# bjzhb666/GS-LoRA

Measured on AMD Instinct MI355X. Metric: forgetting-step images/sec, ViT-P8S8 d6 112px r=8, higher is better.
Workload: dtype fp16

## Files before the change

### gs-lora_amd/csrc/gemm.hip

```cpp
#include <stdlib.h>

#include "gsl_common.h"
#include <type_traits>

using namespace gsl;
#include "gsl_h16.h"
GSL_OPNS_BEGIN

typedef op16x8_t bf16x8_t;
typedef __attribute__((ext_vector_type(4))) float f32x4_t;

struct EpiArgs {
  float alpha;
  const float* bias;
  const void* res;
  const void* aux;
  void* out;
  void* out2;
  int ldo;
  const float* pos;
  const float* cls;
  int T;
  DropCfg drop;
  int M, N;
// ... 2173 lines not shown
      return launch_gemm<GSL_EPI_MUL>(dtype, A1, lda1, W1, ldw1, K1, A2, lda2, W2, ldw2, K2, e, st);
    case GSL_EPI_BIAS_GELU_G8:
      GSL_CHECK_ARG(bias && dtype == GSL_OP16 && (N % 64) == 0, "bias required, bf16 only, N % 64 == 0 (slab-major code tensor)");
      return launch_gemm<GSL_EPI_BIAS_GELU_G8>(dtype, A1, lda1, W1, ldw1, K1, A2, lda2, W2, ldw2, K2, e, st);
    case GSL_EPI_MUL_G8:
      GSL_CHECK_ARG(aux && dtype == GSL_OP16 && (N % 64) == 0, "aux required, bf16 only, N % 64 == 0 (slab-major code tensor)");
      return launch_gemm<GSL_EPI_MUL_G8>(dtype, A1, lda1, W1, ldw1, K1, A2, lda2, W2, ldw2, K2, e, st);
    case GSL_EPI_PATCH:
      GSL_CHECK_ARG(bias && pos && cls && T > 0, "bias/pos/cls/T required");
      return launch_gemm<GSL_EPI_PATCH>(dtype, A1, lda1, W1, ldw1, K1, A2, lda2, W2, ldw2, K2, e, st);
    default: return fail(GSL_ERR_ARG, "gsl_gemm_nt: unknown epilogue%s %ld", "", epilogue);
  }
}

static int gemm_nt_lora_rows(const void* A, int lda, const void* W, int ldw, int K, const void* P, int ldp, const void* Q,
                             int ldq, float lora_scale, void* tout, int ldt, int M, int N, int dtype, int epilogue,
                             const float* bias, const void* res, const void* aux, void* out, void* out2, int ldo,
                             float p_drop, uint64_t seed, uint32_t site, gsl_stream_t s, int mbase);

extern "C" int GSL_ENTRY(gsl_gemm_nt_lora)(const void* A, int lda, const void* W, int ldw, int K, const void* P, int ldp, const void* Q,
                                int ldq, float lora_scale, void* tout, int ldt, int M, int N, int dtype, int epilogue,
                                const float* bias, const void* res, const void* aux, void* out, void* out2, int ldo,
                                float p_drop, uint64_t seed, uint32_t site, gsl_stream_t s) {
  GSL_FORWARD_H16(dtype, h16_gsl_gemm_nt_lora(A, lda, W, ldw, K, P, ldp, Q, ldq, lora_scale, tout, ldt, M, N, dtype, epilogue, bias, res, aux, out,
                                              out2, ldo, p_drop, seed, site, s));
  const bool splittable = (epilogue == GSL_EPI_STORE && !out2) || epilogue == GSL_EPI_BIAS_RES_BF16 || epilogue == GSL_EPI_BIAS_RES_F16;
  const int tail = (splittable && A && W && out && M >= 1024) ? tail_split_rows(M, N, dtype) : 0;
  if (tail > 0) {
    const int head = M - tail;
    const int rc = gemm_nt_lora_rows(A, lda, W, ldw, K, P, ldp, Q, ldq, lora_scale, tout, ldt, head, N, dtype, epilogue, bias, res, aux, out, out2, ldo,
                                     p_drop, seed, site, s, 0);
    if (rc) return rc;
    return gemm_nt_lora_rows(rows_after(A, head, lda, 2), lda, W, ldw, K, P, ldp, Q, ldq, lora_scale, rows_after(tout, head, ldt, 2), ldt, tail, N, dtype,
                             epilogue, bias, rows_after(res, head, ldo, 2), aux, rows_after(out, head, ldo, 2), out2, ldo, p_drop, seed, site, s, head);
  }
  return gemm_nt_lora_rows(A, lda, W, ldw, K, P, ldp, Q, ldq, lora_scale, tout, ldt, M, N, dtype, epilogue, bias, res, aux, out, out2, ldo, p_drop, seed,
                           site, s, 0);
}

static int gemm_nt_lora_rows(const void* A, int lda, const void* W, int ldw, int K, const void* P, int ldp, const void* Q,
                             int ldq, float lora_scale, void* tout, int ldt, int M, int N, int dtype, int epilogue,
                             const float* bias, const void* res, const void* aux, void* out, void* out2, int ldo,
                             float p_drop, uint64_t seed, uint32_t site, gsl_stream_t s, int mbase) {
  if (dtype != GSL_OP16) return fail(GSL_ERR_UNSUPPORTED, "gsl_gemm_nt_lora: bf16 / fp16 operands only (f32 parity mode uses gsl_gemm_nt with a K segment)%s %ld", "", dtype);
  GSL_CHECK_ARG(M > 0 && N > 0 && (N % 4) == 0 && K > 0 && (K % 64) == 0, "M,N>0, N%4==0, K%64==0");
  GSL_CHECK_ARG(A && W && P && Q && out, "null operand");
// ... 152 lines not shown
```

### gs-lora_amd/csrc/gsl_common.h

```cpp
#pragma once
#include <hip/hip_runtime.h>
#include <stdint.h>
#include <stdio.h>
#include <string.h>

#include "../../include/gslora_hip.h"

namespace gsl {

extern thread_local char g_err[512];
inline int fail(int code, const char* fmt, const char* a = "", long b = 0, long c = 0) {
  snprintf(g_err, sizeof(g_err), fmt, a, b, c);
  return code;
}
#define GSL_CHECK_ARG(cond, msg)                                                        \
  do {                                                                                  \
    if (!(cond)) return gsl::fail(GSL_ERR_ARG, "%s: argument check failed: " msg " (%ld,%ld)", __func__, 0, 0); \
  } while (0)
inline int check_launch(const char* what) {
  hipError_t e = hipGetLastError();
  if (e != hipSuccess) {
    snprintf(g_err, sizeof(g_err), "%s: %s", what, hipGetErrorString(e));
    return GSL_ERR_LAUNCH;
  }
// ... 195 lines not shown
__device__ __forceinline__ void drop_mul4(const DropCfg& d, uint64_t idx, float m[4]) {
  drop_mul4_w(d, d.thr ? drop_w0(d.key, idx >> 1) : 0u, m);
}

__device__ __forceinline__ float gelu_f(float x) { return 0.5f * x * (1.0f + erff(x * 0.70710678118654752f)); }
__device__ __forceinline__ float gelu_grad_f(float x) {
  const float cdf = 0.5f * (1.0f + erff(x * 0.70710678118654752f));
  const float pdf = 0.39894228040143268f * expf(-0.5f * x * x);
  return cdf + x * pdf;
}

__device__ __forceinline__ void gelu_pair_fast(float a, float& g, float& gp) {
  const float t = __builtin_amdgcn_rcpf(fmaf(fabsf(a), 0.3275911f * 0.70710678118654752f, 1.0f));
  const float e = __builtin_amdgcn_exp2f((a * a) * -0.72134752044448170f);
  const float ph = t * fmaf(t, fmaf(t, fmaf(t, fmaf(t, 0.5f * 1.061405429f, 0.5f * -1.453152027f), 0.5f * 1.421413741f), 0.5f * -0.284496736f),
                            0.5f * 0.254829592f);
  const float cdf = 0.5f + copysignf(fmaf(-ph, e, 0.5f), a);
  g = a * cdf;
  gp = fmaf(a * 0.39894228040143268f, e, cdf);
}

inline hipStream_t as_stream(gsl_stream_t s) { return reinterpret_cast<hipStream_t>(s); }

}
```

### gs-lora_amd/csrc/lora.hip

```cpp
#include "gsl_common.h"

using namespace gsl;

constexpr int LG_ROWS = 64;
constexpr int LG_FAN = 32;

template <typename T> struct LgVec;
template <> struct LgVec<bf16_t> {
  static constexpr int V = 8;
  static __device__ __forceinline__ void ld(const bf16_t* p, float v[8]) {
    const uint4 t = *reinterpret_cast<const uint4*>(p);
    v[0] = __uint_as_float(t.x << 16); v[1] = __uint_as_float(t.x & 0xffff0000u);
    v[2] = __uint_as_float(t.y << 16); v[3] = __uint_as_float(t.y & 0xffff0000u);
    v[4] = __uint_as_float(t.z << 16); v[5] = __uint_as_float(t.z & 0xffff0000u);
    v[6] = __uint_as_float(t.w << 16); v[7] = __uint_as_float(t.w & 0xffff0000u);
  }
};
template <> struct LgVec<f16_t> {
  static constexpr int V = 8;
  static __device__ __forceinline__ void ld(const f16_t* p, float v[8]) {
    const uint4 t = *reinterpret_cast<const uint4*>(p);
    unpack2h(t.x, v[0], v[1]); unpack2h(t.y, v[2], v[3]); unpack2h(t.z, v[4], v[5]); unpack2h(t.w, v[6], v[7]);
  }
};
// ... 366 lines not shown
  }
  lg_plan(M, N, V, R, CG, bx, nsplit, rps);
  const int RP = 256 / CG;
  const size_t red_bytes = (size_t)(RP - 1) * CG * V * R * sizeof(float);
  float* part2 = ws + (size_t)nsplit * N * R;
#define LAUNCH(TT, RR)                                                                                                   \
  hipLaunchKernelGGL((lora_grad_partial_kernel<TT, RR>), dim3(bx, nsplit), dim3(256), red_bytes, st, (const TT*)Y, ldy, (const TT*)U, \
                     ldu, ws, M, N, rps, CG)
  if (dtype == GSL_BF16) { if (R == 8) LAUNCH(bf16_t, 8); else LAUNCH(bf16_t, 16); }
  else if (dtype == GSL_F16) { if (R == 8) LAUNCH(f16_t, 8); else LAUNCH(f16_t, 16); }
  else { if (R == 8) LAUNCH(float, 8); else LAUNCH(float, 16); }
#undef LAUNCH
  int rc = check_launch("gsl_lora_grad(partial)");
  if (rc) return rc;
  const int tot = N * R;
  int nslab = (nsplit + LG_FAN - 1) / LG_FAN;
  if (nslab == 1) { part2 = ws; nslab = nsplit; }
  else hipLaunchKernelGGL(lora_grad_reduce1_kernel, dim3((tot + 255) / 256, nslab), dim3(256), 0, st, ws, part2, tot, nsplit);
  if (R == 8) hipLaunchKernelGGL(lora_grad_reduce2_kernel<8>, dim3((tot + 255) / 256), dim3(256), 0, st, part2, G, gsn, gsj, N, r, nslab, accumulate, gscale);
  else hipLaunchKernelGGL(lora_grad_reduce2_kernel<16>, dim3((tot + 255) / 256), dim3(256), 0, st, part2, G, gsn, gsj, N, r, nslab, accumulate, gscale);
  return check_launch("gsl_lora_grad(reduce)");
}

__global__ __launch_bounds__(256) void gnorm_partial_kernel(const float* __restrict__ flat, const int64_t* __restrict__ toff,
                                                            const int64_t* __restrict__ tnumel, float* __restrict__ partial) {
  fp16_sat_on();
  __shared__ float sm[16];
  const int t = blockIdx.x, sp = blockIdx.y;
  const int64_t n = tnumel[t];
  const float* p = flat + toff[t];
  const int64_t chunk = ((n + GSL_NORM_SPLIT - 1) / GSL_NORM_SPLIT + 3) & ~(int64_t)3;
  const int64_t b = sp * chunk, e = min(n, b + chunk);
  float acc = 0.f;
  const bool al = ((reinterpret_cast<uintptr_t>(p + b) & 15) == 0);
  if (al) {
    const int64_t n4 = (e > b) ? (e - b) / 4 : 0;
    const float4* p4 = reinterpret_cast<const float4*>(p + b);
    for (int64_t i = threadIdx.x; i < n4; i += blockDim.x) {
      const float4 v = p4[i];
      acc += v.x * v.x + v.y * v.y + v.z * v.z + v.w * v.w;
    }
    for (int64_t i = b + n4 * 4 + threadIdx.x; i < e; i += blockDim.x) acc += p[i] * p[i];
  } else {
    for (int64_t i = b + threadIdx.x; i < e; i += blockDim.x) acc += p[i] * p[i];
  }
  const float tot = block_sum(acc, sm);
// ... 285 lines not shown
```

### gs-lora_amd/csrc/norm.hip

```cpp
#include "gsl_common.h"

using namespace gsl;

template <int NPL>
struct RowIO {
  static constexpr int VEC = (NPL % 4 == 0) ? 4 : 1;
  static constexpr int NV = NPL / VEC;
  static __device__ __forceinline__ int idx(int lane, int c, int i) { return (c * 64 + lane) * VEC + i; }
  template <typename T>
  static __device__ __forceinline__ void load(const T* row, int lane, float v[NPL]) {
#pragma unroll
    for (int c = 0; c < NV; ++c) {
      if constexpr (VEC == 4) Elem<T>::ld4(row + (c * 64 + lane) * 4, &v[c * 4]);
      else v[c] = Elem<T>::ld(row + c * 64 + lane);
    }
  }
  template <typename T>
  static __device__ __forceinline__ void store(T* row, int lane, const float v[NPL]) {
#pragma unroll
    for (int c = 0; c < NV; ++c) {
      if constexpr (VEC == 4) Elem<T>::st4(row + (c * 64 + lane) * 4, &v[c * 4]);
      else Elem<T>::st(row + c * 64 + lane, v[c]);
    }
  }
// ... 54 lines not shown
#pragma unroll
      for (int i = 0; i < NPL; ++i) am = fmaxf(am, fabsf(gy[i]));
    }
#pragma unroll
    for (int i = 0; i < NPL; ++i) {
      xv[i] = (xv[i] - mu) * rs;
      gy[i] *= g[i];
      s1 += gy[i];
      s2 += gy[i] * xv[i];
    }
    const float c1 = wave_sum(s1) * (1.0f / D), c2 = wave_sum(s2) * (1.0f / D);
#pragma unroll
    for (int i = 0; i < NPL; ++i) gy[i] = rs * (gy[i] - c1 - xv[i] * c2);
    if (dres && (cls_T == 0 || (row % cls_T) == 0)) {
      float r[NPL];
      IO::load(dres + (size_t)(cls_T ? row / cls_T : row) * ios, lane, r);
#pragma unroll
      for (int i = 0; i < NPL; ++i) gy[i] += r[i];
    }
    if (gmax) {
#pragma unroll
      for (int i = 0; i < NPL; ++i) am = fmaxf(am, fabsf(gy[i]));
    }
    IO::store(dx + (size_t)row * (cls_T ? (long)D : ios), lane, gy);
    if (dxb) {
      if (drop.thr) {
#pragma unroll
        for (int c = 0; c < IO::NV; ++c) {
          if constexpr (IO::VEC == 4) {
            float dm[4];
            drop_mul4(drop, (uint64_t)row * drop_row_stride + IO::idx(lane, c, 0), dm);
#pragma unroll
            for (int i = 0; i < 4; ++i) gy[c * 4 + i] *= dm[i];
          } else {
            gy[c] *= drop_mul(drop, (uint64_t)row * drop_row_stride + IO::idx(lane, c, 0));
          }
        }
      }
      IO::store(dxb + (size_t)row * D, lane, gy);
    }
  }
  if (gmax) {
    am = wave_max(am);
    if (lane == 0 && !(am <= *gmax)) atomicMax(reinterpret_cast<unsigned int*>(gmax), __float_as_uint(am));
  }
}

// ... 132 lines not shown
    case 256: return CALL(4);                                                               \
    case 512: return CALL(8);                                                               \
    case 768: return CALL(12);                                                              \
    case 1024: return CALL(16);                                                             \
    default: return fail(GSL_ERR_UNSUPPORTED, "%s: unsupported LayerNorm width %ld", __func__, (long)(D)); \
  }

extern "C" int gsl_layernorm_fwd(const void* x, long x_row_stride, const float* gamma, const float* beta, float eps,
                                 void* y, float* mean, float* rstd, int M, int D, int dtype, int x_dtype, gsl_stream_t s) {
  GSL_CHECK_ARG(x && gamma && beta && mean && rstd && M > 0, "null/size");
  GSL_CHECK_ARG(dtype == GSL_F32 || dtype == GSL_BF16 || dtype == GSL_F16, "dtype");
  GSL_CHECK_ARG(x_dtype == GSL_F32 || ((x_dtype == GSL_BF16 || x_dtype == GSL_F16) && dtype == GSL_BF16) || (x_dtype == GSL_F16 && dtype == GSL_F16),
                "x dtype (a 16-bit stream only in a 16-bit mode; bf16 stream only with bf16 operands)");
  GSL_CHECK_ARG((x_row_stride % 4) == 0, "row stride alignment");
#define CALL(N) ln_fwd_launch<N>(x, x_row_stride, gamma, beta, eps, y, mean, rstd, M, dtype, x_dtype, as_stream(s))
  GSL_DISPATCH_D(D, CALL)
#undef CALL
}

extern "C" int gsl_layernorm_bwd(const void* dy, const void* x, long x_row_stride, const float* gamma, const float* mean,
                                 const float* rstd, const void* dres, void* dx, long io_row_stride, void* dxb, int M, int D,
                                 int dtype, int stream_dtype, int x_dtype, float p_drop, uint64_t seed, uint32_t site,
                                 long drop_row_stride, int dres_cls_T, float* gmax, gsl_stream_t s) {
  GSL_CHECK_ARG(dy && x && gamma && mean && rstd && dx && M > 0, "null/size");
  GSL_CHECK_ARG(dtype == GSL_F32 || dtype == GSL_BF16 || dtype == GSL_F16, "dtype");
  GSL_CHECK_ARG(stream_dtype == GSL_F32 || (stream_dtype == dtype && dtype != GSL_F32), "stream dtype (f32, or the operand format of a 16-bit mode)");
  GSL_CHECK_ARG(x_dtype == GSL_F32 || ((x_dtype == GSL_BF16 || x_dtype == GSL_F16) && dtype == GSL_BF16) || (x_dtype == GSL_F16 && dtype == GSL_F16),
                "x dtype (a 16-bit stream only in a 16-bit mode; bf16 stream only with bf16 operands)");
  GSL_CHECK_ARG((x_row_stride % 4) == 0, "row stride alignment");
  GSL_CHECK_ARG(dres_cls_T >= 0 && (dres_cls_T == 0 || (dres && dres != dx)), "dres_cls_T: compact dres, out of place");
  const DropCfg drop = make_drop(p_drop, seed, site);
  const long ios = io_row_stride > 0 ? io_row_stride : D, drs = drop_row_stride > 0 ? drop_row_stride : D;
  GSL_CHECK_ARG((ios % 4) == 0, "io row stride alignment");
#define CALL(N) ln_bwd_launch<N>(dy, x, x_row_stride, gamma, mean, rstd, dres, dx, ios, dxb, M, dtype, stream_dtype, x_dtype, drop, drs, dres_cls_T, gmax, as_stream(s))
  GSL_DISPATCH_D(D, CALL)
#undef CALL
}

extern "C" int gsl_layernorm_fwd_lora(const void* x, long x_row_stride, const float* gamma, const float* beta, float eps, void* y,
                                      float* mean, float* rstd, int M, int D, const void* P, int ldp, float alpha, void* u,
                                      gsl_stream_t s) {
  GSL_CHECK_ARG(x && gamma && beta && y && mean && rstd && P && u && M > 0, "null/size");
  GSL_CHECK_ARG(D == 512 || D == 768, "width (512 or 768)");
  GSL_CHECK_ARG((x_row_stride % 8) == 0 && (ldp % 8) == 0 && ldp >= D, "row stride alignment");
  const int grid = min((M + 63) / 64, 256 * 4);
  if (D == 512)
    hipLaunchKernelGGL((ln_fwd_lora_kernel<16>), dim3(grid), dim3(256), 0, as_stream(s), (const bf16_t*)x, x_row_stride, gamma, beta, eps,
// ... 7 lines not shown
```

### gs-lora_amd/gslora_hip/ops.py

```python
import ctypes

import torch

from . import _lib as L

ATTN_MAX_T = 1025


def check_num_tokens(model, T):
    if T > ATTN_MAX_T:
        raise NotImplementedError(f"{model}: this geometry gives {T} tokens per image; the gs-lora_amd attention kernels take at most "
                                  f"{ATTN_MAX_T} (GSL_ATTN_MAX_T: a 32 x 32 patch grid plus the cls token)")


DT = {torch.float32: L.F32, torch.bfloat16: L.BF16, torch.float16: L.F16}


def _p(t):
    return None if t is None else t.data_ptr()


def _stream():
    return torch.cuda.current_stream().cuda_stream

# ... 269 lines not shown
    _need(x, gamma, beta)
    mean = torch.empty(M, device=x.device, dtype=torch.float32)
    rstd = torch.empty(M, device=x.device, dtype=torch.float32)
    L.check(L.load().gsl_layernorm_fwd(_p(x), row_stride, _p(gamma), _p(beta), float(eps), None, _p(mean), _p(rstd), M, D,
                                       code(dtype), code(x.dtype), _stream()), "gsl_layernorm_fwd(stats)")
    return mean, rstd


def layernorm_fwd_lora(x, row_stride, M, D, gamma, beta, eps, P, alpha, pad=64):
    _need(x, gamma, beta, P)
    if x.dtype != torch.bfloat16 or P.dtype != torch.bfloat16 or P.shape[0] < 16 or P.shape[1] != D or pad != 64:
        raise ValueError("layernorm_fwd_lora: bf16 x, P [>= 16, D] bf16, 64-column u")
    y = torch.empty(M, D, device=x.device, dtype=torch.bfloat16)
    u = torch.empty(M, pad, device=x.device, dtype=torch.bfloat16)
    mean = torch.empty(M, device=x.device, dtype=torch.float32)
    rstd = torch.empty(M, device=x.device, dtype=torch.float32)
    L.check(L.load().gsl_layernorm_fwd_lora(_p(x), row_stride, _p(gamma), _p(beta), float(eps), _p(y), _p(mean), _p(rstd), M, D,
                                            _p(P), P.stride(0), float(alpha), _p(u), _stream()), "gsl_layernorm_fwd_lora")
    return y, mean, rstd, u


@_profiled("ln_bwd", lambda dy, *a, **k: (dy.shape[0], dy.shape[1], 0, 0))
def layernorm_bwd(dy, x, row_stride, gamma, mean, rstd, dres, want_copy=True, p_drop=0.0, seed=0, site=0, dx=None,
                  io_row_stride=0, drop_row_stride=0, dres_cls_T=0, gmax=None):
    _need(dy, x, gamma, mean, rstd)
    M, D = dy.shape
    sdt = dx.dtype if dx is not None else (dres.dtype if dres is not None else torch.float32)
    own_dx = dx is None
    if dx is None:
        _need(dres)
        dx = torch.empty(M, D, device=dy.device, dtype=sdt)
    elif dres is not None and dres.dtype != dx.dtype:
        raise RuntimeError("layernorm_bwd: dres and dx must share one dtype")
    alias = bool(want_copy) and float(p_drop) == 0.0 and sdt == dy.dtype and own_dx and not io_row_stride
    dxb = torch.empty(M, D, device=dy.device, dtype=dy.dtype) if (want_copy and not alias) else None
    L.check(L.load().gsl_layernorm_bwd(_p(dy), _p(x), row_stride, _p(gamma), _p(mean), _p(rstd), _p(dres), _p(dx),
                                       int(io_row_stride), _p(dxb), M, D, code(dy.dtype), code(sdt), code(x.dtype), float(p_drop),
                                       int(seed), int(site), int(drop_row_stride), int(dres_cls_T), _p(gmax), _stream()), "gsl_layernorm_bwd")
    return dx, (dx if alias else dxb)


@_profiled("attn_fwd", lambda qkv, B, T, H, *a, **k: (B * T, H * 64, T, H))
def attention_fwd(qkv, B, T, H, scale, layout=0):
    _need(qkv)
    o = torch.empty(B * T, H * 64, device=qkv.device, dtype=qkv.dtype)
    lse = torch.empty(B, H, T, device=qkv.device, dtype=torch.float32)
    L.check(L.load().gsl_attention_fwd(_p(qkv), _p(o), _p(lse), B, T, H, float(scale), code(qkv.dtype), int(layout), _stream()),
            "gsl_attention_fwd")
    return o, lse


@_profiled("attn_bwd", lambda qkv, o, d_o, lse, B, T, H, *a, **k: (B * T, H * 64, T, H))
def attention_bwd(qkv, o, d_o, lse, B, T, H, scale, layout=0):
    _need(qkv, o, d_o, lse)
    dqkv = torch.empty_like(qkv)
    delta = torch.empty(B, H, T, device=qkv.device, dtype=torch.float32)
    L.check(L.load().gsl_attention_bwd(_p(qkv), _p(o), _p(d_o), _p(lse), _p(dqkv), _p(delta), B, T, H, float(scale),
                                       code(qkv.dtype), int(layout), _stream()), "gsl_attention_bwd")
    return dqkv


def attention_fwd_cls(qkv, B, T, H, scale, layout=0, q_cls=None):
# ... 7 lines not shown

def attention_bwd_cls(qkv, o, d_o_cls, lse, B, T, H, scale, layout=0, q_cls=None):
    _need(qkv, o, d_o_cls, lse, q_cls)
    nw = 2 if layout == 2 else 3
    dqkv = torch.empty(B * T, nw * H * 64, device=qkv.device, dtype=qkv.dtype)
    dq = torch.empty(B, H * 64, device=qkv.device, dtype=qkv.dtype) if layout == 2 else None
    compact = o.shape[0] == B and lse.dim() == 2
    L.check(L.load().gsl_attention_bwd_cls(_p(qkv), _p(q_cls), _p(o), _p(d_o_cls), _p(lse), _p(dqkv), _p(dq), B, T, H, float(scale),
                                           code(qkv.dtype), int(layout), 1 if compact else 0, _stream()), "gsl_attention_bwd_cls")
    return (dqkv, dq) if layout == 2 else dqkv




def lora_grad(Y, U, G, gsn, gsj, r, accumulate=True, gscale=None):
    if not (Y.is_cuda and U.is_cuda and Y.stride(1) == 1 and U.stride(1) == 1):
        raise RuntimeError("lora_grad: operands must be CUDA tensors with unit column stride")
    M, N = Y.shape
    lib = L.load()
    need = lib.gsl_lora_grad_ws_elems(M, N, r)
    ws = _workspace((Y.device.index,), need, Y.device, floor=1 << 22)
    L.check(lib.gsl_lora_grad(_p(Y), Y.stride(0), _p(U), U.stride(0), G.data_ptr(), gsn, gsj, M, N, r, code(Y.dtype),
                              1 if accumulate else 0, _p(ws), _p(gscale), _stream()), "gsl_lora_grad")


class _LgradDesc(ctypes.Structure):
    _fields_ = [("Y", ctypes.c_void_p), ("ldy", ctypes.c_long), ("U", ctypes.c_void_p), ("ldu", ctypes.c_int), ("M", ctypes.c_int),
                ("N", ctypes.c_int), ("r", ctypes.c_int), ("accumulate", ctypes.c_int), ("pad_", ctypes.c_int), ("G", ctypes.c_void_p),
                ("gsn", ctypes.c_long), ("gsj", ctypes.c_long)]


def lora_grad_batchable(Y, U, r):
    return (Y.dtype in (torch.bfloat16, torch.float16) and U.dtype == Y.dtype and Y.is_cuda and Y.stride(1) == 1 and U.stride(1) == 1
            and Y.shape[1] % 256 == 0 and Y.stride(0) % 8 == 0 and U.stride(0) % 8 == 0 and U.stride(0) >= 16 and 1 <= r <= 16
            and Y.data_ptr() % 16 == 0 and U.data_ptr() % 16 == 0)


def lora_grad_batch(entries, gscale=None):
    if not entries:
        return
    assert ctypes.sizeof(_LgradDesc) == 72
    arr = (_LgradDesc * len(entries))()
    for k, (Y, U, G, gsn, gsj, r, acc) in enumerate(entries):
        arr[k] = _LgradDesc(Y.data_ptr(), Y.stride(0), U.data_ptr(), U.stride(0), Y.shape[0], Y.shape[1], r, 1 if acc else 0, 0,
                            G.data_ptr(), gsn, gsj)
    lib = L.load()
# ... 443 lines not shown
```

### gs-lora_amd/gslora_hip/vit_runner.py

```python
import os

import torch

from . import _lib as L
from . import ops

PADK = 64
OP16 = (torch.bfloat16, torch.float16)
SITE_EMB = 1_000_000
GRAD_STREAM_BF16 = os.environ.get("GSLORA_GRAD_STREAM", "bf16").lower() != "f32"
FWD_STREAM = os.environ.get("GSLORA_FWD_STREAM", "f16").lower()
if FWD_STREAM not in ("f16", "bf16", "f32"):
    raise ValueError(f"GSLORA_FWD_STREAM must be f16, bf16 or f32, not {FWD_STREAM!r}")
GP8 = os.environ.get("GSLORA_GP8", "1") != "0"

FUSE_LORA_GRAD = True
TAIL_CLS = True
QSPLIT = True
INK_MIN_ROWS = 8192
LN1_FOLD = os.environ.get("GSLORA_LN1_FOLD", "1") != "0"
GRAD_TARGET_EXP = int(os.environ.get("GSLORA_GRAD_TARGET_EXP", "0"))
if GRAD_TARGET_EXP and not 4 <= GRAD_TARGET_EXP <= 15:
    raise ValueError(f"GSLORA_GRAD_TARGET_EXP={GRAD_TARGET_EXP}: 0 (default) or 4 .. 15")
INK_SMALL = True
LGRAD_BATCH_MAX_ROWS = 1 << 30
LN_LORA = False
QKV_HEAD_MAJOR = True


class BlockSpec:
    __slots__ = ("ln1", "qkv_w", "qkv_b", "out", "ln2", "l1", "l2", "qkv_lora")

    def __init__(self, ln1, qkv_w, qkv_b, out, ln2, l1, l2, qkv_lora=None):
        self.ln1, self.qkv_w, self.qkv_b, self.out, self.ln2, self.l1, self.l2 = ln1, qkv_w, qkv_b, out, ln2, l1, l2
        self.qkv_lora = qkv_lora

    def lora_params(self):
        if self.qkv_lora is not None:
            return (self.qkv_lora.lora_A, self.qkv_lora.lora_B)
        return (self.l1.lora_A, self.l1.lora_B, self.l2.lora_A, self.l2.lora_B)


LINEAR_HEADS = ("linear", "softmax")


class ModelSpec:
    __slots__ = ("patch_size", "num_tokens", "dim", "heads", "attn_scale", "ln_eps", "dropout_p", "emb_dropout_p", "lora_rank",
                 "patch_w", "patch_is_conv", "patch_b", "cls", "pos", "blocks", "final_ln", "head_kind", "head_w", "head_b",
                 "cos_s", "cos_m", "easy_margin", "lora_site", "pool", "patch_kernel", "patch_stride", "patch_pad", "image_size")
# ... 265 lines not shown
        if ents and (tab is None or tab[2] != len(ents)):
            if tab is not None:
                self._retired.append(tab[0])
            t, mx = ops.pack_desc_table([(e["param"], *e["geom"], 1.0, e["out"]) for e in ents], ents[0]["dev"])
            tab = self._pack_tables[dtype] = (t, mx, len(ents))
        return tab

    def _zeros(self, n, dev):
        z = self._wcache.get(("zeros", n, dev))
        if z is None:
            z = self._wcache[("zeros", n, dev)] = torch.zeros(n, device=dev, dtype=torch.float32)
        return z

    def lora_in_kernel(self, dtype, rows, N=None):
        if dtype not in OP16 or self._rank > 16:
            return False
        if rows >= INK_MIN_ROWS:
            return True
        if N is None or not INK_SMALL:
            return False
        t256 = ((rows + 255) // 256) * ((N + 255) // 256)
        t128 = ((rows + 127) // 128) * ((N + 127) // 128)
        return (rows < 1024 or t256 < 128) and t128 <= 256

    def ensure_bucket(self, spec=None):
        spec = spec or self.model.hip_spec()
        self._rank = spec.lora_rank
        if spec.lora_rank <= 0:
            return None
        layers = [blk.lora_params() for blk in spec.blocks]
        if self.bucket is None or not self.bucket.valid() or any(a is not b for a, b in zip(self.bucket.params, (p for g in layers for p in g))):
            self.bucket = LoraBucket(layers)
            self._lcache.clear()
            self._retired.extend(t[0] for t in self._pack_tables.values())
            self._retired.extend(e["out"] for e in self._packs.values())
            self._packs.clear()
            self._pack_tables.clear()
        return self.bucket

    def forward(self, img, label, save):
        head_only = save == "head"
        save = save is True
        c, parts, u8tab, label = self._fwd_prepare(img, label, save)
        sp = c.sp
        x = self._fwd_patch(c, parts, u8tab)
        stash = []
# ... 126 lines not shown
                                                               self.lora_pack(f"A1_{i}", l1.lora_A, "A_rows", dt), s_lora)
        else:
            xn2, mean2, rstd2 = ops.layernorm_fwd(x1, D, Mr, D, n2.weight.detach(), n2.bias.detach(), c.eps, dt)
        if lora_on and (abs(l1.scaling * r - 1.0) > 1e-9 or abs(l2.scaling * r - 1.0) > 1e-9):
            raise NotImplementedError("gs-lora_amd: the fused LoRA path uses scaling = 1 / r (lora_alpha = 1, the only value GS-LoRA "
                                      f"passes); got scaling {l1.scaling} / {l2.scaling} for r = {r}")
        u1 = u2 = u1c = None
        h = torch.empty(Mr, mlp, device=dev, dtype=dt)
        gp8 = GP8 and dt in OP16 and save and mlp % 64 == 0
        epi_gelu = L.EPI_BIAS_GELU_G8 if gp8 else L.EPI_BIAS_GELU
        gp = torch.empty(Mr, mlp, device=dev, dtype=torch.uint8 if gp8 else dt) if save else None
        if lora_on:
            if Mr < INK_MIN_ROWS and not ln_u1 and self.lora_in_kernel(dt, Mr, mlp):
                u1 = torch.empty(Mr, PADK, device=dev, dtype=dt)
                ops.gemm_nt_lora(xn2, self.w(f"w1_{i}", l1.weight, dt), self.lora_pack(f"A1_{i}", l1.lora_A, "A_rows16", dt),
                                 self.lora_pack(f"B1_{i}", l1.lora_B, "B_cols32", dt), s_lora, u1, h, epilogue=epi_gelu,
                                 bias=l1.bias.detach(), out2=gp, p_drop=p_drop, seed=seed, site=(4 * i + 1) | sflag, tag="ffn1")
            else:
                if ln_u1:
                    u1 = u1_ln
                else:
                    u1 = torch.empty(Mr, PADK, device=dev, dtype=dt)
                    u1c = torch.empty(Mr, 16, device=dev, dtype=dt) if (save and dt in OP16 and r <= 16 and Mr >= INK_MIN_ROWS) else None
                    c.gemm(xn2, self.lora_pack(f"A1_{i}", l1.lora_A, "A_rows", dt), u1, alpha=s_lora, out2=u1c)
                c.gemm(xn2, self.w(f"w1_{i}", l1.weight, dt), h, epilogue=epi_gelu, A2=u1,
                            W2=self.lora_pack(f"B1_{i}", l1.lora_B, "B_cols", dt), bias=l1.bias.detach(), out2=gp,
                            p_drop=p_drop, seed=seed, site=(4 * i + 1) | sflag, tag="ffn1")
            u2 = torch.empty(Mr, PADK, device=dev, dtype=dt)
            if not self.lora_in_kernel(dt, Mr, D):
                c.gemm(h, self.lora_pack(f"A2_{i}", l2.lora_A, "A_rows", dt), u2, alpha=s_lora)
        else:
            c.gemm(xn2, self.w(f"w1_{i}", l1.weight, dt), h, epilogue=epi_gelu, bias=l1.bias.detach(),
                        out2=gp, p_drop=p_drop, seed=seed, site=(4 * i + 1) | sflag)
        x2 = torch.empty(Mr, D, device=dev, dtype=c.xdt)
        if lora_on and self.lora_in_kernel(dt, Mr, D):
            ops.gemm_nt_lora(h, self.w(f"w2_{i}", l2.weight, dt), self.lora_pack(f"A2_{i}", l2.lora_A, "A_rows16", dt),
                             self.lora_pack(f"B2_{i}", l2.lora_B, "B_cols32", dt), s_lora, u2, x2, epilogue=c.epi_res,
                             bias=l2.bias.detach(), res=x1, p_drop=p_drop, seed=seed, site=(4 * i + 2) | sflag)
        else:
            c.gemm(h, self.w(f"w2_{i}", l2.weight, dt), x2, epilogue=c.epi_res, A2=u2,
                        W2=self.lora_pack(f"B2_{i}", l2.lora_B, "B_cols", dt) if lora_on else None,
                        bias=l2.bias.detach(), res=x1, p_drop=p_drop, seed=seed, site=(4 * i + 2) | sflag)
        return x2, (dict(mean2=mean2, rstd2=rstd2, xn2=xn2, u1=u1, u1c=u1c, h=h, gp=gp, u2=u2, lora_on=lora_on) if save else None)

    def _fwd_head(self, c, x, label):
        sp, B, D, hn = c.sp, c.B, c.D, c.sp.final_ln
        Th = x.shape[0] // B
# ... 42 lines not shown
        for i in reversed(range(nl)):
            st, blk = saved["layers"][i], sp.blocks[i]
            sparse = (i == nl - 1) and sp.pool == "cls"
            gather = sparse and not st["tail"]
            dxn2 = (self._bwd_ffn_frozen if c.attn_site else self._bwd_ffn_lora)(c, i, blk, st, dxb, gather)
            if dxn2 is None:
                break
            dx1, dx1b = self._bwd_ln2(c, i, blk, st, dxn2, dx, gather)
            del dxn2
            d_o = torch.empty(dx1b.shape[0], c.H * 64, device=c.dev, dtype=c.dt)
            c.gemm(dx1b, self.wT(f"wo{i}", blk.out.weight, c.dt), d_o)
            if c.attn_site:
                dqkv = self._bwd_attention(c, st, d_o, sparse)
                del d_o, dx1b
                dxn1 = self._bwd_qkv_lora(c, i, blk, st, dqkv)
                del dqkv
                if dxn1 is None:
                    break
            else:
                dxn1 = self._bwd_qkv_frozen(c, i, blk, st, d_o, sparse)
                del d_o, dx1b
            dx, dxb = ops.layernorm_bwd(dxn1, st["x"], c.D, blk.ln1.weight.detach(), st["mean1"], st["rstd1"], dx1,
                                        p_drop=c.p_drop, seed=c.seed, site=(4 * (i - 1) + 2) | c.sflag,
                                        dres_cls_T=c.T if sparse else 0, gmax=c.gmax)
            saved["layers"][i] = None
        if not c.attn_site and not torch.cuda.is_current_stream_capturing():
            self.build_pack_tables(c.dt)

    def _bwd_head(self, c, saved, dlogits, demb):
        sp, dt = c.sp, c.dt
        if dlogits is not None:
            dlogits = dlogits.contiguous().float()
        if demb is not None:
            demb = demb.contiguous().float()
        if dlogits is not None and saved["Wn"] is None:
            raise RuntimeError("backward through logits requires a forward with labels")
        c.gscale = self._loss_scale_state(saved["x_last"].device) if dt == torch.float16 else None
        self._guard_on = c.gscale is not None
        c.gmax = c.gscale[2:] if c.gscale is not None else None
        linear_head = sp.head_kind in LINEAR_HEADS
        margin = {}
        if sp.head_kind == "arcface":
            margin = dict(head_kind="arcface", m=sp.cos_m, easy_margin=sp.easy_margin, cos_y=saved["cos_y"], label=saved["label"])
        return (ops.head_bwd_margin if margin else ops.head_bwd)(
            dlogits, demb, saved["x_last"], c.B, saved["Th"], c.D, sp.final_ln.weight.detach(), saved["meanh"], saved["rstdh"],
            saved["emb"], saved["Wn"], 1.0 if linear_head else sp.cos_s, dt, p_drop=c.p_drop, seed=c.seed,
            site=(4 * (len(saved["layers"]) - 1) + 2) | c.sflag, linear=linear_head, pool_mean=(sp.pool == "mean"),
# ... 35 lines not shown
        da = torch.empty(Mrows, mlp, device=dev, dtype=dt)
        fused_grads = ink and FUSE_LORA_GRAD and Mrows >= INK_MIN_ROWS
        if fused_grads:
            ops.gemm_nt_lora_mulgrad(dyb, self.wT(f"w2_{i}", l2.weight, dt), self.lora_pack(f"B2_{i}", l2.lora_B, "BT_rows16", dt),
                                     self.lora_pack(f"A2_{i}", l2.lora_A, "AT_cols32", dt), s_lora, v2, da, gp,
                                     (u1c if u1c is not None else u1), gv[id(l1.lora_B)], (r, 1), h, gv[id(l2.lora_A)], (1, mlp), r, tag="ffn2dx", p_drop=p_drop,
                                     gscale=c.gscale)
        elif ink:
            ops.gemm_nt_lora(dyb, self.wT(f"w2_{i}", l2.weight, dt), self.lora_pack(f"B2_{i}", l2.lora_B, "BT_rows16", dt),
                             self.lora_pack(f"A2_{i}", l2.lora_A, "AT_cols32", dt), s_lora, v2, da, epilogue=epi_mul, aux=gp, p_drop=p_drop)
        else:
            c.gemm(dyb, self.lora_pack(f"B2_{i}", l2.lora_B, "BT_rows", dt), v2, alpha=s_lora)
            c.gemm(dyb, self.wT(f"w2_{i}", l2.weight, dt), da, epilogue=epi_mul, A2=v2,
                        W2=self.lora_pack(f"A2_{i}", l2.lora_A, "AT_cols", dt), aux=gp, p_drop=p_drop)
        self._lgrad(c, dyb, u2, gv[id(l2.lora_B)], r, 1, r)
        if not fused_grads:
            self._lgrad(c, h, v2, gv[id(l2.lora_A)], 1, mlp, r)
        v1 = torch.empty(Mrows, PADK, device=dev, dtype=dt)
        dxn2 = None
        if ink1 and i > 0:
            dxn2 = torch.empty(Mrows, D, device=dev, dtype=dt)
            ops.gemm_nt_lora(da, self.wT(f"w1_{i}", l1.weight, dt), self.lora_pack(f"B1_{i}", l1.lora_B, "BT_rows16", dt),
                             self.lora_pack(f"A1_{i}", l1.lora_A, "AT_cols32", dt), s_lora, v1, dxn2)
        else:
            c.gemm(da, self.lora_pack(f"B1_{i}", l1.lora_B, "BT_rows", dt), v1, alpha=s_lora)
        if not fused_grads:
            self._lgrad(c, da, u1, gv[id(l1.lora_B)], r, 1, r)
        self._lgrad(c, xn2, v1, gv[id(l1.lora_A)], 1, D, r)
        self._grads_done(c, i)
        if i == 0:
            self._flush(c)
            return None
        if dxn2 is None:
            dxn2 = torch.empty(Mrows, D, device=dev, dtype=dt)
            c.gemm(da, self.wT(f"w1_{i}", l1.weight, dt), dxn2, A2=v1,
                        W2=self.lora_pack(f"A1_{i}", l1.lora_A, "AT_cols", dt))
        return dxn2

    def _bwd_ffn_frozen(self, c, i, blk, st, dyb, gather):
        dt, l1, l2 = c.dt, blk.l1, blk.l2
        if st["uq"] is None:
            raise RuntimeError("backward with merged LoRA weights is undefined (model.train() un-merges)")
        mlp = l1.weight.shape[0]
        gp = _gp_rows(c, st["gp"], mlp) if gather else st["gp"]
        da = torch.empty(dyb.shape[0], mlp, device=c.dev, dtype=dt)
        c.gemm(dyb, self.wT(f"w2_{i}", l2.weight, dt), da, epilogue=L.EPI_MUL_G8 if gp.dtype == torch.uint8 else L.EPI_MUL, aux=gp,
# ... 48 lines not shown
```

Measured before the change: 45690.

## Add streaming LoRA down-projection kernel with LDS-resident P and skip unused LN-bwd dx

Adds a dedicated rank-16 down-projection kernel that keeps the small P matrix in LDS, streams X rows through a deep register prefetch queue and uses MFMA 16x16x32 instructions. It replaces the general GEMM for the FFN1 forward and FFN1 backward LoRA down-projections, which should cut tile-shape waste on a skinny N=16 output. Separately, layernorm backward can now skip writing dx when only the operand copy is needed, as in the last layer-1 call, saving one store pass. The new kernel is persistent-grid with a hardcoded CU count and zeroes the padding columns of u, so correctness depends on the packed layouts matching.

```diff
diff --git a/gs-lora_amd/csrc/gemm.hip b/gs-lora_amd/csrc/gemm.hip
--- a/gs-lora_amd/csrc/gemm.hip
+++ b/gs-lora_amd/csrc/gemm.hip
@@ -2219,6 +2219,12 @@
                                 int ldq, float lora_scale, void* tout, int ldt, int M, int N, int dtype, int epilogue,
                                 const float* bias, const void* res, const void* aux, void* out, void* out2, int ldo,
                                 float p_drop, uint64_t seed, uint32_t site, gsl_stream_t s) {
+#ifndef GSL_OP_F16
+  if (!W && !Q && !out && N == 0) {
+    GSL_CHECK_ARG(tout && ldt == 64 && epilogue == GSL_EPI_STORE && !bias && !res && !aux, "t-only form: tout dense [M,64], STORE, no bias / res / aux");
+    return gsl::lora_down_launch(A, lda, P, ldp, K, lora_scale, tout, out2, M, dtype, s);
+  }
+#endif
   GSL_FORWARD_H16(dtype, h16_gsl_gemm_nt_lora(A, lda, W, ldw, K, P, ldp, Q, ldq, lora_scale, tout, ldt, M, N, dtype, epilogue, bias, res, aux, out,
                                               out2, ldo, p_drop, seed, site, s));
   const bool splittable = (epilogue == GSL_EPI_STORE && !out2) || epilogue == GSL_EPI_BIAS_RES_BF16 || epilogue == GSL_EPI_BIAS_RES_F16;
diff --git a/gs-lora_amd/csrc/gsl_common.h b/gs-lora_amd/csrc/gsl_common.h
--- a/gs-lora_amd/csrc/gsl_common.h
+++ b/gs-lora_amd/csrc/gsl_common.h
@@ -241,4 +241,6 @@
 
 inline hipStream_t as_stream(gsl_stream_t s) { return reinterpret_cast<hipStream_t>(s); }
 
-}
+int lora_down_launch(const void* X, long ldx, const void* P, int ldp, int K, float alpha, void* u, void* u16, int M, int dtype, gsl_stream_t s);
+
+}
diff --git a/gs-lora_amd/csrc/lora.hip b/gs-lora_amd/csrc/lora.hip
--- a/gs-lora_amd/csrc/lora.hip
+++ b/gs-lora_amd/csrc/lora.hip
@@ -412,6 +412,99 @@
   return check_launch("gsl_lora_grad(reduce)");
 }
 
+constexpr int LD_CUS = 256;
+static inline int ld_kcap(int K) { return K <= 512 ? 512 : (K <= 1024 ? 1024 : (K <= 2048 ? 2048 : 3072)); }
+static inline int ld_blocks_per_cu(int K) { const int c = ld_kcap(K); return c == 512 ? 7 : (c == 1024 ? 4 : (c == 2048 ? 2 : 1)); }
+
+template <int KCAP, bool F16>
+__global__ __launch_bounds__(256) void lora_down_kernel(const bf16_t* __restrict__ X, long ldx, const bf16_t* __restrict__ P, int ldp, int K,
+                                                        float alpha, bf16_t* __restrict__ u, bf16_t* __restrict__ u16, int M) {
+  fp16_sat_on();
+  constexpr int DEPTH = KCAP > 1024 ? 16 : 8;
+  __shared__ __attribute__((aligned(16))) bf16_t sP[16 * (KCAP + 8)];
+  const int PLD = K + 8, KC = K >> 3;
+  for (int i0 = 0; i0 < 16 * KC; i0 += 4 * 256) {
+    uint4 t[4];
+    int at[4];
+#pragma unroll
+    for (int q = 0; q < 4; ++q) {
+      const int i = min(i0 + q * 256 + (int)threadIdx.x, 16 * KC - 1), j = i / KC, c = i - j * KC;
+      at[q] = j * PLD + c * 8;
+      t[q] = *reinterpret_cast<const uint4*>(P + (size_t)j * ldp + c * 8);
+    }
+#pragma unroll
+    for (int q = 0; q < 4; ++q) *reinterpret_cast<uint4*>(&sP[at[q]]) = t[q];
+  }
+  __syncthreads();
+  const int lane = threadIdx.x & 63, r = lane & 15, kc = lane >> 4;
+  const int wave = __builtin_amdgcn_readfirstlane((int)(threadIdx.x >> 6));
+  const int KS = K >> 5, ngrp = (M + 15) >> 4, gstride = (int)gridDim.x * 4;
+  int cg = (int)blockIdx.x * 4 + wave;
+  if (cg >= ngrp) return;
+  const int KSP = (KS + DEPTH - 1) / DEPTH * DEPTH;
+  auto rowptr = [&](int g) { return X + (size_t)min(g * 16 + r, M - 1) * ldx + kc * 8; };
+  int lg = cg, ls = 0;
+  const bf16_t* lp = rowptr(lg);
+  auto issue = [&](uint4& dst) {
+    dst = *reinterpret_cast<const uint4*>(lp + min(ls, KS - 1) * 32);
+    if (ls + 1 < KSP) ++ls;
+    else if (lg + gstride < ngrp) { lg += gstride; ls = 0; lp = rowptr(lg); }
+  };
+  uint4 v[DEPTH];
+#pragma unroll
+  for (int j = 0; j < DEPTH; ++j) issue(v[j]);
+  const bf16_t* pfrag = sP + r * PLD + kc * 8;
+  for (; cg < ngrp; cg += gstride) {
+    lg_f32x4_t acc = {0.f, 0.f, 0.f, 0.f};
+    for (int s = 0; s < KSP; s += DEPTH) {
+#pragma unroll
+      for (int j = 0; j < DEPTH; ++j) {
+        if (s + j < KS) {
+          union { uint4 q4; lg_bf16x8_t v; lg_f16x8_t w; } xf, pf;
+          pf.q4 = *reinterpret_cast<const uint4*>(pfrag + (s + j) * 32);
+          xf.q4 = v[j];
+          if constexpr (F16) acc = __builtin_amdgcn_mfma_f32_16x16x32_f16(pf.w, xf.w, acc, 0, 0, 0);
+          else acc = __builtin_amdgcn_mfma_f32_16x16x32_bf16(pf.v, xf.v, acc, 0, 0, 0);
+        }
+        issue(v[j]);
+      }
+    }
+    const int row = cg * 16 + r;
+    if (row < M) {
+      const float a0 = acc[0] * alpha, a1 = acc[1] * alpha, a2 = acc[2] * alpha, a3 = acc[3] * alpha;
+      const uint2 o = F16 ? make_uint2(pack2h(a0, a1), pack2h(a2, a3)) : make_uint2(pack2bf(a0, a1), pack2bf(a2, a3));
+      bf16_t* pu = u + (size_t)row * 64;
+      *reinterpret_cast<uint2*>(pu + kc * 4) = o;
+      *reinterpret_cast<uint4*>(pu + 16 + kc * 8) = make_uint4(0u, 0u, 0u, 0u);
+      if (kc < 2) *reinterpret_cast<uint4*>(pu + 48 + kc * 8) = make_uint4(0u, 0u, 0u, 0u);
+      if (u16) *reinterpret_cast<uint2*>(u16 + (size_t)row * 16 + kc * 4) = o;
+    }
+    __builtin_amdgcn_s_waitcnt(0x0F70);
+  }
+}
+
+int gsl::lora_down_launch(const void* X, long ldx, const void* P, int ldp, int K, float alpha, void* u, void* u16, int M, int dtype,
+                          gsl_stream_t s) {
+  GSL_CHECK_ARG(X && P && u && M > 0 && K > 0, "null/size");
+  GSL_CHECK_ARG(dtype == GSL_BF16 || dtype == GSL_F16, "dtype: bf16 or fp16 operands");
+  GSL_CHECK_ARG((K % 32) == 0 && ldx >= K && (ldx % 8) == 0 && ldp >= K && (ldp % 8) == 0, "K % 32 == 0, row strides >= K and multiples of 8");
+  GSL_CHECK_ARG((reinterpret_cast<uintptr_t>(X) % 16) == 0 && (reinterpret_cast<uintptr_t>(P) % 16) == 0 && (reinterpret_cast<uintptr_t>(u) % 16) == 0 &&
+                (reinterpret_cast<uintptr_t>(u16) % 8) == 0, "16-byte aligned X / P / u, 8-byte aligned u16");
+  if (K > 3072) return fail(GSL_ERR_UNSUPPORTED, "%s: K = %ld is beyond the 3072 columns the LDS image of P holds", __func__, (long)K);
+  const int grid = min((M + 63) / 64, LD_CUS * ld_blocks_per_cu(K));
+#define GSL_LD(CAP, FF) hipLaunchKernelGGL((lora_down_kernel<CAP, FF>), dim3(grid), dim3(256), 0, as_stream(s), (const bf16_t*)X, ldx, (const bf16_t*)P, ldp, K, alpha, (bf16_t*)u, (bf16_t*)u16, M)
+#define GSL_LD_F(CAP) do { if (dtype == GSL_F16) GSL_LD(CAP, true); else GSL_LD(CAP, false); } while (0)
+  switch (ld_kcap(K)) {
+    case 512: GSL_LD_F(512); break;
+    case 1024: GSL_LD_F(1024); break;
+    case 2048: GSL_LD_F(2048); break;
+    default: GSL_LD_F(3072); break;
+  }
+#undef GSL_LD_F
+#undef GSL_LD
+  return check_launch("gsl_gemm_nt_lora(lora_down)");
+}
+
 __global__ __launch_bounds__(256) void gnorm_partial_kernel(const float* __restrict__ flat, const int64_t* __restrict__ toff,
                                                             const int64_t* __restrict__ tnumel, float* __restrict__ partial) {
   fp16_sat_on();
diff --git a/gs-lora_amd/csrc/norm.hip b/gs-lora_amd/csrc/norm.hip
--- a/gs-lora_amd/csrc/norm.hip
+++ b/gs-lora_amd/csrc/norm.hip
@@ -100,7 +100,7 @@
 #pragma unroll
       for (int i = 0; i < NPL; ++i) am = fmaxf(am, fabsf(gy[i]));
     }
-    IO::store(dx + (size_t)row * (cls_T ? (long)D : ios), lane, gy);
+    if (dx) IO::store(dx + (size_t)row * (cls_T ? (long)D : ios), lane, gy);
     if (dxb) {
       if (drop.thr) {
 #pragma unroll
@@ -279,7 +279,7 @@
                                  const float* rstd, const void* dres, void* dx, long io_row_stride, void* dxb, int M, int D,
                                  int dtype, int stream_dtype, int x_dtype, float p_drop, uint64_t seed, uint32_t site,
                                  long drop_row_stride, int dres_cls_T, float* gmax, gsl_stream_t s) {
-  GSL_CHECK_ARG(dy && x && gamma && mean && rstd && dx && M > 0, "null/size");
+  GSL_CHECK_ARG(dy && x && gamma && mean && rstd && (dx || dxb) && M > 0, "null/size (dx may be NULL only when dxb is given)");
   GSL_CHECK_ARG(dtype == GSL_F32 || dtype == GSL_BF16 || dtype == GSL_F16, "dtype");
   GSL_CHECK_ARG(stream_dtype == GSL_F32 || (stream_dtype == dtype && dtype != GSL_F32), "stream dtype (f32, or the operand format of a 16-bit mode)");
   GSL_CHECK_ARG(x_dtype == GSL_F32 || ((x_dtype == GSL_BF16 || x_dtype == GSL_F16) && dtype == GSL_BF16) || (x_dtype == GSL_F16 && dtype == GSL_F16),
diff --git a/gs-lora_amd/gslora_hip/ops.py b/gs-lora_amd/gslora_hip/ops.py
--- a/gs-lora_amd/gslora_hip/ops.py
+++ b/gs-lora_amd/gslora_hip/ops.py
@@ -315,22 +315,24 @@
 
 @_profiled("ln_bwd", lambda dy, *a, **k: (dy.shape[0], dy.shape[1], 0, 0))
 def layernorm_bwd(dy, x, row_stride, gamma, mean, rstd, dres, want_copy=True, p_drop=0.0, seed=0, site=0, dx=None,
-                  io_row_stride=0, drop_row_stride=0, dres_cls_T=0, gmax=None):
+                  io_row_stride=0, drop_row_stride=0, dres_cls_T=0, gmax=None, want_dx=True):
     _need(dy, x, gamma, mean, rstd)
     M, D = dy.shape
     sdt = dx.dtype if dx is not None else (dres.dtype if dres is not None else torch.float32)
     own_dx = dx is None
+    if not want_dx and not (want_copy and own_dx):
+        raise RuntimeError("layernorm_bwd: want_dx=False returns the operand copy alone (want_copy, no dx buffer of the caller's)")
+    alias = bool(want_copy) and float(p_drop) == 0.0 and sdt == dy.dtype and own_dx and not io_row_stride
     if dx is None:
         _need(dres)
-        dx = torch.empty(M, D, device=dy.device, dtype=sdt)
+        dx = torch.empty(M, D, device=dy.device, dtype=sdt) if (want_dx or alias) else None
     elif dres is not None and dres.dtype != dx.dtype:
         raise RuntimeError("layernorm_bwd: dres and dx must share one dtype")
-    alias = bool(want_copy) and float(p_drop) == 0.0 and sdt == dy.dtype and own_dx and not io_row_stride
     dxb = torch.empty(M, D, device=dy.device, dtype=dy.dtype) if (want_copy and not alias) else None
     L.check(L.load().gsl_layernorm_bwd(_p(dy), _p(x), row_stride, _p(gamma), _p(mean), _p(rstd), _p(dres), _p(dx),
                                        int(io_row_stride), _p(dxb), M, D, code(dy.dtype), code(sdt), code(x.dtype), float(p_drop),
                                        int(seed), int(site), int(drop_row_stride), int(dres_cls_T), _p(gmax), _stream()), "gsl_layernorm_bwd")
-    return dx, (dx if alias else dxb)
+    return (dx if want_dx else None), (dx if alias else dxb)
 
 
 @_profiled("attn_fwd", lambda qkv, B, T, H, *a, **k: (B * T, H * 64, T, H))
@@ -384,6 +386,24 @@
     ws = _workspace((Y.device.index,), need, Y.device, floor=1 << 22)
     L.check(lib.gsl_lora_grad(_p(Y), Y.stride(0), _p(U), U.stride(0), G.data_ptr(), gsn, gsj, M, N, r, code(Y.dtype),
                               1 if accumulate else 0, _p(ws), _p(gscale), _stream()), "gsl_lora_grad")
+
+
+LORA_DOWN_MAX_BLOCKS = 2048
+
+
+@_profiled(None, lambda X, P, *a, **k: (X.shape[0], 16, X.shape[1], 0))
+def lora_down(X, P, u, alpha=1.0, u16=None, tag=None):
+    _need(X, P, rows_ok=True)
+    _need(u, u16)
+    M, K = X.shape
+    if X.dtype not in (torch.bfloat16, torch.float16) or P.dtype != X.dtype or u.dtype != X.dtype or (u16 is not None and u16.dtype != X.dtype):
+        raise RuntimeError("lora_down: X, P, u and u16 share one 16-bit operand dtype (bf16 or fp16)")
+    if tuple(P.shape) != (16, K) or tuple(u.shape) != (M, 64) or (u16 is not None and tuple(u16.shape) != (M, 16)):
+        raise RuntimeError(f"lora_down: P [16, K], u [M, 64], u16 [M, 16] for X [{M}, {K}]; got {tuple(P.shape)}, {tuple(u.shape)}, "
+                           f"{None if u16 is None else tuple(u16.shape)}")
+    L.check(L.load().gsl_gemm_nt_lora(_p(X), X.stride(0), None, 0, K, _p(P), P.stride(0), None, 0, float(alpha), _p(u), 64, M, 0, code(X.dtype),
+                                      L.EPI_STORE, None, None, None, None, _p(u16), 0, 0.0, 0, 0, _stream()), "gsl_gemm_nt_lora(t only)")
+    return u
 
 
 class _LgradDesc(ctypes.Structure):
diff --git a/gs-lora_amd/gslora_hip/vit_runner.py b/gs-lora_amd/gslora_hip/vit_runner.py
--- a/gs-lora_amd/gslora_hip/vit_runner.py
+++ b/gs-lora_amd/gslora_hip/vit_runner.py
@@ -25,6 +25,7 @@
 INK_SMALL = True
 LGRAD_BATCH_MAX_ROWS = 1 << 30
 LN_LORA = False
+LORA_DOWN_STREAM = True
 QKV_HEAD_MAJOR = True
 
 
@@ -336,6 +337,9 @@
         t256 = ((rows + 255) // 256) * ((N + 255) // 256)
         t128 = ((rows + 127) // 128) * ((N + 127) // 128)
         return (rows < 1024 or t256 < 128) and t128 <= 256
+
+    def lora_down_stream(self, dtype, rows, K):
+        return LORA_DOWN_STREAM and dtype in OP16 and self._rank <= 16 and rows >= INK_MIN_ROWS and K % 32 == 0 and K <= 3072
 
     def ensure_bucket(self, spec=None):
         spec = spec or self.model.hip_spec()
@@ -508,7 +512,10 @@
                 else:
                     u1 = torch.empty(Mr, PADK, device=dev, dtype=dt)
                     u1c = torch.empty(Mr, 16, device=dev, dtype=dt) if (save and dt in OP16 and r <= 16 and Mr >= INK_MIN_ROWS) else None
-                    c.gemm(xn2, self.lora_pack(f"A1_{i}", l1.lora_A, "A_rows", dt), u1, alpha=s_lora, out2=u1c)
+                    if self.lora_down_stream(dt, Mr, D):
+                        ops.lora_down(xn2, self.lora_pack(f"A1_{i}", l1.lora_A, "A_rows16", dt), u1, alpha=s_lora, u16=u1c)
+                    else:
+                        c.gemm(xn2, self.lora_pack(f"A1_{i}", l1.lora_A, "A_rows", dt), u1, alpha=s_lora, out2=u1c)
                 c.gemm(xn2, self.w(f"w1_{i}", l1.weight, dt), h, epilogue=epi_gelu, A2=u1,
                             W2=self.lora_pack(f"B1_{i}", l1.lora_B, "B_cols", dt), bias=l1.bias.detach(), out2=gp,
                             p_drop=p_drop, seed=seed, site=(4 * i + 1) | sflag, tag="ffn1")
@@ -597,7 +604,8 @@
                 del d_o, dx1b
             dx, dxb = ops.layernorm_bwd(dxn1, st["x"], c.D, blk.ln1.weight.detach(), st["mean1"], st["rstd1"], dx1,
                                         p_drop=c.p_drop, seed=c.seed, site=(4 * (i - 1) + 2) | c.sflag,
-                                        dres_cls_T=c.T if sparse else 0, gmax=c.gmax)
+                                        dres_cls_T=c.T if sparse else 0, gmax=c.gmax,
+                                        want_dx=c.attn_site or i != 1)
             saved["layers"][i] = None
         if not c.attn_site and not torch.cuda.is_current_stream_capturing():
             self.build_pack_tables(c.dt)
@@ -679,6 +687,8 @@
             dxn2 = torch.empty(Mrows, D, device=dev, dtype=dt)
             ops.gemm_nt_lora(da, self.wT(f"w1_{i}", l1.weight, dt), self.lora_pack(f"B1_{i}", l1.lora_B, "BT_rows16", dt),
                              self.lora_pack(f"A1_{i}", l1.lora_A, "AT_cols32", dt), s_lora, v1, dxn2)
+        elif self.lora_down_stream(dt, Mrows, mlp):
+            ops.lora_down(da, self.lora_pack(f"B1_{i}", l1.lora_B, "BT_rows16", dt), v1, alpha=s_lora)
         else:
             c.gemm(da, self.lora_pack(f"B1_{i}", l1.lora_B, "BT_rows", dt), v1, alpha=s_lora)
         if not fused_grads:
```

Result: no change. 45940 (median of 6 runs) (+0.5%).
